# ohsnyt/bzip2-rust

Measured on NVIDIA B200. Metric: compress_MBps_level9_byte_identical, higher is better.
Workload: dtype u8

## Files before the change

bzip2_rust_b200/csrc/common.cuh:

```cuda
#pragma once
#include <cuda_runtime.h>
#include <stdint.h>
#include <stddef.h>
#include <mutex>
#include <string>
#include <vector>
#include <new>
#include "../../include/bz2b200.h"

typedef uint8_t u8;
typedef uint16_t u16;
typedef uint32_t u32;
typedef uint64_t u64;

#define BZ_CHECK(call)                                                                     \
    do {                                                                                   \
        cudaError_t e_ = (call);                                                           \
        if (e_ != cudaSuccess) {                                                           \
            ctx->fail(#call, e_, __FILE__, __LINE__);                                      \
            return BZ2B200_E_CUDA;                                                         \
        }                                                                                  \
    } while (0)

#define BZ_API_TRY try {
// ... 35 lines not shown
constexpr int BZ_TILE = BZ_THREADS * BZ_IPT;
constexpr int BZ_GROUP = 50;
constexpr int BZ_MAXSYM = 258;

struct Batch {
    int nblk;
    u32 stride;
    u32 tiles;
    u32 max_n;
    int nbits;
    const u8 *T;
    const u32 *len;
    u64 total_n;
};

enum KernelId { K_RADIX_HIST0, K_RADIX_SCAN, K_RADIX_SCATTER0, K_REF_PATH, K_BYTE_HIST, K_DIGIT_SCAN, K_SWEEP_GATHER, K_SWEEP_CARRY, K_SWEEP_LIST, K_INIT_RANKS, K_LIST_KEY, K_LIST_REFINE, K_REFINE_LOCAL, K_BWT_OUT, K_USED, K_MTF_SUMMARY, K_MTF_SCAN, K_MTF_EMIT, K_HUF_INIT, K_HUF_SELECT, K_HUF_LENGTHS, K_HUF_GBITS, K_HUF_LAYOUT, K_HUF_EMIT, K_RLE_SCAN, K_RLE_CHAIN, K_RLE_EMIT, K_CRC_PIECES, K_CRC_FINAL, K_CONCAT, K_FOOTER, K_DEC_MISC, K_DEC_MAGIC, K_DEC_HEADER, K_DEC_JUMPS, K_DEC_BOUNDS, K_DEC_SYMS, K_DEC_CHUNKS, K_DEC_EXPAND, K_DEC_CHUNK_SCAN, K_IBWT_CHASE, K_IBWT_RANK, K_IBWT_WRITE, K_DEC_RLE1_COUNT, K_DEC_RLE1_WRITE, K_COUNT };
static const char *const kKernelNames[] = { "k_radix_hist0", "k_radix_scan", "k_radix_scatter0", "k_ref_path", "k_byte_hist", "k_digit_scan", "k_sweep_gather", "k_sweep_carry", "k_sweep_list", "k_init_ranks", "k_list_key", "k_list_refine", "k_refine_local", "k_bwt_out", "k_used", "k_mtf_summary", "k_mtf_scan", "k_mtf_emit", "k_huf_init", "k_huf_select", "k_huf_lengths", "k_huf_gbits", "k_huf_layout", "k_huf_emit", "k_rle_scan", "k_rle_chain", "k_rle_emit", "k_crc_pieces", "k_crc_final", "k_concat", "k_footer", "k_dec_misc", "k_dec_find_magic", "k_dec_header", "k_dec_jumps", "k_dec_bounds", "k_dec_syms", "k_dec_chunks", "k_dec_expand", "k_dec_chunk_scan", "k_ibwt_chase", "k_ibwt_rank", "k_ibwt_write", "k_dec_rle1_count", "k_dec_rle1_write" };

struct KStat { double ms = 0; u64 launches = 0; u64 bytes = 0; };
struct PendingEv { int id; u64 bytes; cudaEvent_t a, b; };

struct Arrival {
    std::vector<cudaEvent_t> *ev;
    size_t chunk;
    size_t win_off;
    size_t waited;
};

struct ShardPlan {
    bool scanned = false;
    const u8 *d_win = nullptr; size_t win_lo = 0, win_len = 0, n_total = 0; int level = 0;
    bool planned = false;
// ... 215 lines not shown
```

bzip2_rust_b200/csrc/rle1.cu:

```cuda
#include "common.cuh"
#include <algorithm>
#include <stdlib.h>

namespace {

constexpr u32 CRC_POLY = 0x04C11DB7u;
constexpr int PIECE = 1024;
constexpr u32 NOQ = 0xFFFFFFFFu;

struct BlockRec {
    u32 s, e;
    u32 re;
    u32 g_last;
    u32 out_re;
    u32 out_g;
    u32 out_len;
    u32 last;
};

__host__ __device__ inline u32 gf_mul(u32 a, u32 b) {
    u32 r = 0;
    for (int i = 31; i >= 0; i--) {
        r = (r << 1) ^ ((r & 0x80000000u) ? CRC_POLY : 0u);
        if ((b >> i) & 1u) r ^= a;
// ... 48 lines not shown
        if (!((need >> lane) & 1u)) { v.a = -1; v.c = 0; }
#pragma unroll
        for (int o = 16; o; o >>= 1) {
            v.a = max(v.a, __shfl_xor_sync(0xffffffffu, v.a, o));
            v.c += __shfl_xor_sync(0xffffffffu, v.c, o);
        }
        ex.a = max(ex.a, v.a); ex.c += v.c;
        if (incm) break;
        hi -= 32;
    }
    Pair inc; inc.a = max(ex.a, agg.a); inc.c = ex.c + agg.c;
    if (lane == 0) st_vol64(st + t, pair_pack(2, inc));
    return ex;
}

struct ScanArgs {
    const u8 *x; u32 W;
    u32 *RS, *OUT, *LASTQ;
    u64 *st1, *st2;
    u32 *ticket;
};

constexpr int SC_IPT = 16;
constexpr int SC_TILE = BZ_THREADS * SC_IPT;

#ifndef BZ_SCAN_MINB
#define BZ_SCAN_MINB 5
#endif
__global__ void __launch_bounds__(BZ_THREADS, BZ_SCAN_MINB) k_rle_scan(ScanArgs a) {
    __shared__ u32 s_tile;
    __shared__ int wsi[8];
    __shared__ u32 wsu[8];
    __shared__ Pair s_ex1, s_ex2;
    const int tid = threadIdx.x;
    if (tid == 0) s_tile = atomicAdd(a.ticket, 1u);
    __syncthreads();
    const u32 t = s_tile, W = a.W;
    const u32 i0 = t * SC_TILE + tid * SC_IPT;
    u32 v[6];
    {
        uintptr_t addr = (uintptr_t)(a.x + i0) - 4;
        const u32 *gw = (const u32 *)(addr & ~(uintptr_t)3);
        const u32 mis = (u32)(addr & 3);
        long long j = (long long)i0 - 4 - (long long)mis;
        u32 w[7];
#pragma unroll
        for (int k = 0; k < 7; k++) {
            long long jk = j + 4 * k;
// ... 6 lines not shown
    int last = -1; u32 bdmask = 0;
#pragma unroll
    for (int r = 0; r < SC_IPT; r++) {
        u32 i = i0 + r;
        if (i < W && (i == 0 || XB(r) != XB(r - 1))) { last = (int)i; bdmask |= 1u << r; }
    }
    int tot1;
    int rs = block_excl_max(last, wsi, tot1);
    if (tid < 32) {
        Pair agg; agg.a = tot1; agg.c = 0;
        Pair ex = pair_lookback(a.st1, t, agg);
        if (tid == 0) s_ex1 = ex;
    }
    __syncthreads();
    rs = max(rs, s_ex1.a);
    u32 qmask = 0, litmask = 0, sum = 0;
    int lq = -1;
    const bool full = i0 + SC_IPT <= W;
    u32 rsv[SC_IPT];
#pragma unroll
    for (int r = 0; r < SC_IPT; r++) {
        u32 i = i0 + r;
        rsv[r] = 0;
        if (i < W) {
            if ((bdmask >> r) & 1u) rs = (int)i;
            rsv[r] = (u32)rs;
            u32 d = i - (u32)rs;
            u32 co = d - (d / 255u) * 255u;
            bool grp;
            if (co >= 3) grp = true;
            else {
                u32 c = XB(r);
                grp = (i - co) + 3 < W;
                if (co < 3) grp = grp && XB(r + 1) == c;
                if (co < 2) grp = grp && XB(r + 2) == c;
                if (co < 1) grp = grp && XB(r + 3) == c;
            }
            if (!grp) { litmask |= 1u << r; sum += 1; }
            else if (co == 0) { qmask |= 1u << r; sum += 5; lq = (int)i; }
        }
    }
    if (full) {
        uint4 *o = (uint4 *)(a.RS + i0);
#pragma unroll
        for (int k = 0; k < 4; k++) o[k] = make_uint4(rsv[4 * k], rsv[4 * k + 1], rsv[4 * k + 2], rsv[4 * k + 3]);
    } else {
#pragma unroll
        for (int r = 0; r < SC_IPT; r++) if (i0 + r < W) a.RS[i0 + r] = rsv[r];
    }
    int tq; u32 ts;
    int q = block_excl_max(lq, wsi, tq);
    u32 o = block_excl_sum(sum, wsu, ts);
    if (tid < 32) {
        Pair agg; agg.a = tq; agg.c = ts;
        Pair ex = pair_lookback(a.st2, t, agg);
        if (tid == 0) s_ex2 = ex;
    }
    __syncthreads();
    q = max(q, s_ex2.a);
    o += s_ex2.c;
    u32 ov[SC_IPT], qv[SC_IPT];
#pragma unroll
    for (int r = 0; r < SC_IPT; r++) {
        if ((qmask >> r) & 1u) q = (int)(i0 + r);
        ov[r] = o; qv[r] = q < 0 ? NOQ : (u32)q;
        o += ((litmask >> r) & 1u) + 5u * ((qmask >> r) & 1u);
        if (i0 + r == W - 1) a.OUT[W] = o;
    }
    if (full) {
        uint4 *po = (uint4 *)(a.OUT + i0), *pq = (uint4 *)(a.LASTQ + i0);
#pragma unroll
        for (int k = 0; k < 4; k++) {
            po[k] = make_uint4(ov[4 * k], ov[4 * k + 1], ov[4 * k + 2], ov[4 * k + 3]);
            pq[k] = make_uint4(qv[4 * k], qv[4 * k + 1], qv[4 * k + 2], qv[4 * k + 3]);
        }
    } else {
#pragma unroll
        for (int r = 0; r < SC_IPT; r++) if (i0 + r < W) { a.OUT[i0 + r] = ov[r]; a.LASTQ[i0 + r] = qv[r]; }
    }
#undef XB
}

struct ChainArgs {
    const u8 *x; const u32 *RS; const u32 *OUT; const u32 *LASTQ;
    u32 W;
    u32 B;
    u32 is_eof;
    u32 max_blocks;
    u32 max_out;
    u32 s0;
    u32 stop_at;
    u32 out_w;
    u32 off_from;
    BlockRec *rec; u32 *nrec; u32 *consumed;
};

__device__ u32 warp_lower_bound(const u32 *OUT, u32 lo, u32 hi, long long target) {
    int lane = threadIdx.x & 31;
    while (hi - lo > 32) {
        u32 step = (hi - lo + 31) / 32;
        u64 pp = (u64)lo + (u64)step * (u32)(lane + 1);
        u32 p = pp > hi ? hi : (u32)pp;
        bool ge = (long long)OUT[p] >= target;
        unsigned bal = __ballot_sync(0xffffffffu, ge);
        int f = __ffs(bal) - 1;
        u64 nh = (u64)lo + (u64)step * (u32)(f + 1);
        u32 new_hi = nh > hi ? hi : (u32)nh;
        u32 new_lo = f == 0 ? lo : lo + step * (u32)f + 1;
        lo = new_lo; hi = new_hi;
    }
    u32 p = lo + (u32)lane;
    bool ge = p <= hi && (long long)OUT[p] >= target;
    unsigned bal = __ballot_sync(0xffffffffu, ge);
    return lo + (u32)(__ffs(bal) - 1);
}

__device__ u32 run_end_from(const u32 *RS, u32 W, u32 s) {
    u32 key = RS[s];
    u32 d = 1;
    while (s + d < W && RS[s + d] == key && d < (1u << 30)) d <<= 1;
    u32 lo = s + (d >> 1) + 1, hi = (s + d < W) ? s + d : W;
    if (d == 1) lo = s + 1;
    while (lo < hi) {
        u32 mid = lo + (hi - lo) / 2;
        if (RS[mid] > key) hi = mid; else lo = mid + 1;
    }
    return lo;
}
__device__ u32 group_end(const u8 *x, u32 W, u32 q) {
    u8 c = x[q];
    u32 p = q + 4, lim = min(W, q + 255);
    while (p < lim && x[p] == c) p++;
    return p;
}
__device__ __forceinline__ u32 exit_cursor(u32 g, long long R) {
    if (R <= 1) return g + 1;
    return (R & 1) ? g + (u32)R : g + (u32)R + 1;
}

enum { PLAN_OK = 0, PLAN_STOP = 1, PLAN_SEARCH = 2 };
template <bool COOP>
__device__ __forceinline__ int plan_block(const ChainArgs &a, u32 s, BlockRec &r) {
    const u32 W = a.W, B = a.B;
    const u32 margin = a.is_eof ? 0u : 1024u;
    r.s = s; r.last = 0;
    u32 re = run_end_from(a.RS, W, s);
    if (!a.is_eof && re + margin > W) return PLAN_STOP;
    u32 Lc = re - s;
    u32 nfull = Lc / 255u, rem = Lc % 255u;
    u32 ng_avail = nfull + (rem >= 4 ? 1u : 0u);
    u32 jmax = (B - 1 + 4) / 5;
    u32 g, out_g;
    bool done = false;
    u32 e = 0;
    if (ng_avail > jmax) {
        g = s + 255u * jmax; out_g = 5u * jmax;
        e = g + 1;
        r.re = re; r.out_re = 0;
        done = true;
    } else {
        g = s + 255u * nfull + (rem >= 4 ? rem : 0u);
        out_g = 5u * ng_avail;
        r.re = re; r.out_re = out_g + (re - g);
    }
    bool has_group_after_off = ng_avail > 0 && g > a.off_from;
    if (!done) {
        long long off = (long long)r.out_re - (long long)a.OUT[re];
        long long target = (long long)B - 1 - off;
        u32 x1;
        u32 lq_m1 = NOQ, lq_p3 = NOQ;
        bool have_m1 = false, have_p3 = false;
        if ((long long)a.out_w < target) x1 = W + 1;
        else {
            long long need = target - (long long)a.OUT[re];
            u64 guess = (u64)re + (u64)(need > 0 ? need : 0);
            bool solved = false;
            if (need <= 0) { x1 = re; solved = true; }
            else if (COOP) {
                const int lane = threadIdx.x & 31;
                const long long wlo = (long long)guess - 15;
                const long long p = wlo + lane;
                const bool inb = p >= (long long)re && p <= (long long)W;
                const u32 o = inb ? a.OUT[p] : 0u;
                const u32 lqv = (p >= 0 && p < (long long)W) ? a.LASTQ[p] : NOQ;
                const unsigned bal = __ballot_sync(0xffffffffu, inb && (long long)o >= target);
                const unsigned inm = __ballot_sync(0xffffffffu, inb);
                if (bal) {
                    const int f = __ffs(bal) - 1;
                    const long long xp = wlo + f;
                    if (xp == (long long)re || (f > 0 && ((inm >> (f - 1)) & 1u))) {
                        x1 = (u32)xp; solved = true;
                        if (f >= 1) { lq_m1 = __shfl_sync(0xffffffffu, lqv, f - 1); have_m1 = true; }
                        const long long hl = (long long)min(x1 + 3, W - 1) - wlo;
                        if (hl >= 0 && hl < 32) { lq_p3 = __shfl_sync(0xffffffffu, lqv, (int)hl); have_p3 = true; }
                    }
                }
            }
            if (!solved) {
                if (guess <= W && (long long)a.OUT[guess] >= target && (long long)a.OUT[guess - 1] < target) x1 = (u32)guess;
                else if (COOP) {
                    u64 g64 = guess > W ? W : guess;
                    u32 lo_w = g64 > (u64)re + 512 ? (u32)g64 - 512u : re;
                    u32 hi_w = g64 + 512 < (u64)W ? (u32)g64 + 512u : W;
                    if ((long long)a.OUT[lo_w] < target && (long long)a.OUT[hi_w] >= target) x1 = warp_lower_bound(a.OUT, lo_w, hi_w, target);
                    else x1 = warp_lower_bound(a.OUT, re, W, target);
                } else {
                    u32 lo = re, hi = W;
                    while (lo < hi) {
                        u32 mid = lo + (hi - lo) / 2;
                        if ((long long)a.OUT[mid] >= target) hi = mid; else lo = mid + 1;
                    }
                    x1 = lo;
                }
            }
        }
        u32 gl = NOQ;
        if (x1 <= W) {
            u32 hiq = min(x1 + 3, W - 1);
            u32 q1_pre = x1 < W ? (have_p3 ? lq_p3 : a.LASTQ[hiq]) : NOQ;
            u32 qp_pre = x1 > re ? (have_m1 ? lq_m1 : a.LASTQ[x1 - 1]) : NOQ;
            if (x1 < W) {
                u32 q1 = q1_pre;
                if (q1 != NOQ && q1 >= x1 && q1 >= re && (long long)a.OUT[q1] + off == (long long)B - 1) {
                    u32 gp = g;
                    if (q1 > 0) {
                        u32 qp = a.LASTQ[q1 - 1];
                        if (qp != NOQ && qp >= re) gp = group_end(a.x, W, qp);
                    }
                    if (((q1 - gp) & 1u) == 1u) gl = q1;
                }
            }
            if (gl == NOQ && x1 > re) {
                u32 qp = qp_pre;
                if (qp != NOQ && qp >= re) gl = qp;
            }
        } else if (W > re) {
            u32 qp = a.LASTQ[W - 1];
            if (qp != NOQ && qp >= re) gl = qp;
        }
        if (gl != NOQ) {
            u32 out_gl = a.OUT[gl];
            g = group_end(a.x, W, gl);
            out_g = (u32)((long long)out_gl + off + 5);
            if (gl >= a.off_from) has_group_after_off = true;
        }
        long long R = (long long)B - (long long)out_g;
        e = exit_cursor(g, R);
    }
    if (a.is_eof) {
        u32 lim = has_group_after_off ? W - 1 : W - 2;
        if (W < 2 || e > lim || e > W) {
            e = W; r.last = 1;
            if (!done) {
                if (W > re) {
                    u32 qp = a.LASTQ[W - 1];
                    if (qp != NOQ && qp >= re) {
                        long long off = (long long)r.out_re - (long long)a.OUT[re];
                        g = group_end(a.x, W, qp);
                        out_g = (u32)((long long)a.OUT[qp] + off + 5);
                    }
                }
            } else {
                g = s + 255u * nfull + (rem >= 4 ? rem : 0u);
                out_g = 5u * ng_avail;
                r.out_re = out_g + (re - g);
            }
        }
    } else if (e + margin > W) {
        return PLAN_STOP;
    }
    r.e = e; r.g_last = g; r.out_g = out_g;
    r.out_len = out_g + (e - g);
    if (r.out_len > a.max_out) return PLAN_STOP;
    return PLAN_OK;
// ... 4 lines not shown
constexpr u32 CH_SEG = 128;
__host__ __device__ inline u32 tab_cap(u32 k) { return 32u * k + 256u; }
__host__ __device__ inline u32 tab_off(u32 k) { return 16u * k * (k - 1u) + 256u * (k - 1u); }
constexpr u32 TAB_ENTRIES = 16u * (CH_SEG + 1) * CH_SEG + 256u * CH_SEG;
constexpr u32 REC_BAD = 0xFFFFFFFFu;

struct ChainState { u32 nb, s, done, hits; };

struct TabArgs {
    ChainArgs a;
    ChainState *state;
    u32 *tlo, *tcnt;
    BlockRec *tab;
};

__device__ u32 lower_bound_out(const u32 *OUT, u32 lo, u32 hi, u64 target) {
    if ((u64)OUT[hi] < target) return hi + 1;
    while (lo < hi) {
        u32 mid = lo + (hi - lo) / 2;
        if ((u64)OUT[mid] >= target) hi = mid; else lo = mid + 1;
    }
    return lo;
}

__global__ void __launch_bounds__(128) k_rle_tab_bounds(TabArgs t) {
    const u32 k = blockIdx.x * 128 + threadIdx.x + 1;
    if (k > CH_SEG) return;
    const ChainState st = *t.state;
    t.tcnt[k] = 0;
    if (st.done || st.s >= t.a.W) return;
    const u32 W = t.a.W, B = t.a.B;
    const u64 base = t.a.OUT[st.s];
    u32 lo = lower_bound_out(t.a.OUT, st.s, W, base + (u64)k * (B - 10));
    if (lo > W) return;
    u32 hi = lower_bound_out(t.a.OUT, lo, W, base + (u64)k * (B + 15) + 1);
    if (hi > W) hi = W;
    u32 cap = tab_cap(k);
    if (hi - lo + 1 > cap) {
        u32 c = lower_bound_out(t.a.OUT, lo, hi, base + (u64)k * B + (5ull * k) / 2);
        u32 from = c > lo + cap / 2 ? c - cap / 2 : lo;
        if (from + cap - 1 > hi) from = hi + 1 - cap;
        lo = from; hi = from + cap - 1;
    }
    t.tlo[k] = lo; t.tcnt[k] = hi - lo + 1;
}

__global__ void __launch_bounds__(128) k_rle_tab_fill(TabArgs t) {
    const u32 k = blockIdx.y + 1;
    const u32 j = blockIdx.x * 128 + threadIdx.x;
    if (j >= t.tcnt[k]) return;
    const u32 s = t.tlo[k] + j;
    BlockRec r;
    r.out_len = REC_BAD;
    if (s < t.a.W) {
        ChainArgs a = t.a;
        a.out_w = a.OUT[a.W];
        if (plan_block<false>(a, s, r) != PLAN_OK) r.out_len = REC_BAD;
    }
    t.tab[tab_off(k) + j] = r;
}

__global__ void __launch_bounds__(32) k_rle_chain(TabArgs t) {
    ChainArgs a = t.a;
    const int lane = threadIdx.x;
    const u32 W = a.W;
    ChainState st = *t.state;
    if (st.done) return;
    a.out_w = a.OUT[W];
    u32 s = st.s, nb = st.nb, hits = st.hits;
    u32 span = a.B;
    bool finished = true;
    for (u32 k = 0;; k++) {
        if (!(s < W && s < a.stop_at && nb < a.max_blocks)) break;
        if (k > CH_SEG) { finished = false; break; }
        BlockRec r;
        bool have = false;
        if (t.tab && k >= 1) {
            u32 lo = t.tlo[k], cnt = t.tcnt[k];
            if (s >= lo && s - lo < cnt) {
                const uint4 *src = (const uint4 *)(t.tab + tab_off(k) + (s - lo));
                uint4 q0 = src[0], q1 = src[1];
                r.s = q0.x; r.e = q0.y; r.re = q0.z; r.g_last = q0.w; r.out_re = q1.x; r.out_g = q1.y; r.out_len = q1.z; r.last = q1.w;
                have = r.out_len != REC_BAD && r.s == s;
                hits += have ? 1u : 0u;
            }
        }
        if (!have) {
            {
                u64 c = (u64)s + (u64)span * (lane < 16 ? 1u : 2u);
                long long p = (long long)c - 1024 + (long long)(lane & 15) * 128;
                if (p >= 0 && (u64)p + 32 < (u64)W) {
                    prefetch_l2(a.OUT + p); prefetch_l2(a.OUT + p + 32); prefetch_l2(a.OUT + p + 64); prefetch_l2(a.OUT + p + 96);
                    prefetch_l2(a.LASTQ + p); prefetch_l2(a.LASTQ + p + 32); prefetch_l2(a.LASTQ + p + 64); prefetch_l2(a.LASTQ + p + 96);
                    prefetch_l2(a.RS + p); prefetch_l2(a.RS + p + 32); prefetch_l2(a.RS + p + 64); prefetch_l2(a.RS + p + 96);
                    prefetch_l2(a.x + p);
                }
            }
            if (plan_block<true>(a, s, r) != PLAN_OK) break;
        }
        if (lane == 0) a.rec[nb] = r;
        nb++;
        span = r.e - s;
        s = r.e;
    }
    if (lane == 0) {
        ChainState o; o.nb = nb; o.s = s; o.done = finished ? 1u : 0u; o.hits = hits;
        *t.state = o;
        *a.nrec = nb; *a.consumed = s;
    }
}

__global__ void __launch_bounds__(BZ_THREADS) k_rle_emit(const u8 *x, u32 W, const u32 *RS, const u32 *OUT,
                                                         const BlockRec *rec, u8 *T, u32 *len, u32 stride) {
    u32 k = blockIdx.y;
    BlockRec r = rec[k];
    u32 span = r.e - r.s;
    u32 base = blockIdx.x * BZ_TILE;
    if (base >= span) return;
    if (blockIdx.x == 0 && threadIdx.x == 0) len[k] = r.out_len;
    u8 *out = T + (size_t)k * stride;
    long long off = (long long)r.out_re - (long long)OUT[min(r.re, W)];
#pragma unroll 4
    for (int q = 0; q < BZ_IPT; q++) {
        u32 rel = base + q * BZ_THREADS + threadIdx.x;
        if (rel >= span) continue;
        u32 i = r.s + rel;
        u8 c = x[i];
        if (i >= r.g_last) {
            out[r.out_g + (i - r.g_last)] = c;
        } else if (i < r.re) {
            u32 j = (i - r.s) / 255u, cs = r.s + j * 255u;
            u32 cl = min(255u, r.re - cs);
            if (cl >= 4) {
                if (i == cs) {
                    u8 *o = out + 5u * j;
                    o[0] = c; o[1] = c; o[2] = c; o[3] = c; o[4] = (u8)(cl - 4);
                }
            } else out[5u * j + (i - cs)] = c;
        } else {
            u32 o0 = OUT[i], o1 = OUT[i + 1];
            u32 o = (u32)((long long)o0 + off);
            if (o1 - o0 == 1u) out[o] = c;
            else if (o1 != o0) {
                u32 ge = group_end(x, W, i);
                out[o] = c; out[o + 1] = c; out[o + 2] = c; out[o + 3] = c; out[o + 4] = (u8)(ge - i - 4);
            }
        }
    }
}

__global__ void __launch_bounds__(256) k_crc_pieces(const u8 *x, const u32 *spans, u32 span_stride, u32 s0, u32 e0,
                                                    u32 *part, u32 parts_stride, u32 xp ) {
    __shared__ u32 tab[256];
    __shared__ u32 red[256];
    make_crc_table(tab);
    u32 k = blockIdx.y;
    u32 s = spans ? spans[(size_t)k * span_stride] : s0, e = spans ? spans[(size_t)k * span_stride + 1] : e0;
    u32 span = e - s;
    u32 npieces = (span + PIECE - 1) / PIECE;
    u32 p = blockIdx.x * 256 + threadIdx.x;
    __syncthreads();
// ... 51 lines not shown
    do {                                                             \
        ctx->prof_end();                                             \
        cudaError_t e_ = cudaGetLastError();                         \
        if (e_ != cudaSuccess) { ctx->fail("kernel launch", e_, __FILE__, __LINE__); return BZ2B200_E_CUDA; } \
    } while (0)

int bz_rle1_window(bz2b200_ctx *ctx, const u8 *d_x, u32 W, int level, bool is_eof, u32 off_from, u32 max_blocks,
                   Batch &B, u32 *nblocks, u32 *consumed, std::vector<u32> *h_spans, bool plan_only, u32 stop_at,
                   int skip, u32 s0) {
    const bool skip_scan = skip & 1, skip_chain = skip & 2;
    cudaStream_t st = ctx->stream;
    u32 Bsz = (u32)level * 100000u - 19u;
    u32 max_n = Bsz + 8;
    u32 stride = ((max_n + 64 + BZ_TILE - 1) / BZ_TILE) * BZ_TILE;
    u32 tiles = (W + BZ_TILE - 1) / BZ_TILE;
    const size_t W4 = ((size_t)W + 1 + 3) & ~(size_t)3;
    BZ_CHECK(ctx->d_runflag.ensure(W4 * 4 * 3 + 64));
    u32 *RS = ctx->d_runflag.as<u32>();
    u32 *OUT = RS + W4;
    u32 *LASTQ = OUT + W4;
    const size_t state_bytes = ((size_t)tiles * 8 * 2 + 64 + 15) & ~(size_t)15;
    BZ_CHECK(ctx->d_misc.ensure(state_bytes + (size_t)max_blocks * sizeof(BlockRec) + 256));
    u64 *st1 = ctx->d_misc.as<u64>();
    u64 *st2 = st1 + tiles;
    u32 *ticket = (u32 *)(st2 + tiles);
    BlockRec *rec = (BlockRec *)(ctx->d_misc.as<u8>() + state_bytes);
    u32 *d_small = (u32 *)(rec + max_blocks);
    BZ_CHECK(ctx->h_small.ensure(64 + (size_t)max_blocks * sizeof(BlockRec)));

    if (!skip_scan && W > 0) {
        BZ_CHECK(cudaMemsetAsync(st1, 0, state_bytes, st));
        ScanArgs sa;
        sa.x = d_x; sa.W = W; sa.RS = RS; sa.OUT = OUT; sa.LASTQ = LASTQ; sa.st1 = st1; sa.st2 = st2; sa.ticket = ticket;
        if (!ctx->arrival) {
            ctx->prof_begin(K_RLE_SCAN, (u64)W * 13); k_rle_scan<<<tiles, BZ_THREADS, 0, st>>>(sa); LAUNCH_OK();
        } else {
            Arrival &A = *ctx->arrival;
            const size_t nev = A.ev->size();
            u32 launched = 0;
            while (launched < tiles) {
                if (A.waited < nev) { BZ_CHECK(cudaStreamWaitEvent(st, (*A.ev)[A.waited], 0)); A.waited++; }
                size_t have = A.waited >= nev ? (size_t)-1 : A.waited * A.chunk;
                size_t have_win = have > A.win_off ? have - A.win_off : 0;
                u32 upto = have_win >= W ? tiles : (have_win > 64 ? (u32)((have_win - 64) / SC_TILE) : 0u);
                if (upto > launched) {
                    ctx->prof_begin(K_RLE_SCAN, (u64)(upto - launched) * SC_TILE * 13);
                    k_rle_scan<<<upto - launched, BZ_THREADS, 0, st>>>(sa); LAUNCH_OK();
                    launched = upto;
                }
            }
        }
    }
    ChainArgs a;
    a.x = d_x; a.RS = RS; a.OUT = OUT; a.LASTQ = LASTQ; a.W = W; a.B = Bsz; a.is_eof = is_eof ? 1u : 0u;
    a.max_blocks = max_blocks; a.max_out = max_n; a.off_from = off_from; a.stop_at = stop_at; a.s0 = s0;
    a.rec = rec; a.nrec = d_small; a.consumed = d_small + 1;
    if (plan_only && skip_chain) { *nblocks = 0; *consumed = 0; return BZ2B200_OK; }
    if (!skip_chain) {
        static const bool use_tab = [] { const char *e = getenv("BZ2B200_CHAIN_TABLES"); return !e || atoi(e) != 0; }();
        BZ_CHECK(ctx->d_F.ensure(sizeof(ChainState) + 2 * (size_t)(CH_SEG + 1) * 4 + (size_t)TAB_ENTRIES * sizeof(BlockRec) + 256));
        TabArgs t;
        t.a = a;
        t.state = ctx->d_F.as<ChainState>();
        t.tlo = (u32 *)(t.state + 1);
        t.tcnt = t.tlo + (CH_SEG + 1);
        t.tab = use_tab ? (BlockRec *)(((uintptr_t)(t.tcnt + (CH_SEG + 1)) + 15) & ~(uintptr_t)15) : nullptr;
        ChainState st0; st0.nb = 0; st0.s = s0; st0.done = 0; st0.hits = 0;
        BZ_CHECK(cudaMemcpyAsync(t.state, &st0, sizeof st0, cudaMemcpyHostToDevice, st));
        u64 span_in = (u64)W - (u64)(s0 < W ? s0 : W);
// ... 17 lines not shown
    { int bits = 0; u32 v = max_n - 1; while (v) { bits++; v >>= 1; } B.nbits = bits; }
    if (nb == 0) return BZ2B200_OK;
    BZ_CHECK(ctx->d_T.ensure((size_t)nb * stride + 64));
    BZ_CHECK(ctx->d_len.ensure((size_t)nb * 4));
    BZ_CHECK(ctx->d_crc.ensure((size_t)nb * 4));
    BlockRec *hrec = (BlockRec *)(hs + 16);
    BZ_CHECK(cudaMemcpyAsync(hrec, rec, (size_t)nb * sizeof(BlockRec), cudaMemcpyDeviceToHost, st));
    BZ_CHECK(cudaStreamSynchronize(st));
    u32 max_span = 0;
    B.total_n = 0;
    for (u32 k = 0; k < nb; k++) B.total_n += hrec[k].out_len;
    for (u32 k = 0; k < nb; k++) max_span = hrec[k].e - hrec[k].s > max_span ? hrec[k].e - hrec[k].s : max_span;
    if (h_spans) { h_spans->clear(); for (u32 k = 0; k < nb; k++) { h_spans->push_back(hrec[k].s); h_spans->push_back(hrec[k].e); h_spans->push_back(hrec[k].out_len); h_spans->push_back(hrec[k].last); } }
    if (plan_only) return BZ2B200_OK;
    dim3 ge((max_span + BZ_TILE - 1) / BZ_TILE, nb);
    ctx->prof_begin(K_RLE_EMIT, (u64)max_span * nb * 2); k_rle_emit<<<ge, BZ_THREADS, 0, st>>>(d_x, W, RS, OUT, rec, ctx->d_T.as<u8>(), ctx->d_len.as<u32>(), stride);
    LAUNCH_OK();
    u32 max_pieces = (max_span + PIECE - 1) / PIECE;
    u32 parts_stride = (max_pieces + 255) / 256;
    BZ_CHECK(ctx->d_agg2.ensure((size_t)nb * parts_stride * 4 + 64));
    u32 xp = gf_pow_x8(PIECE), xp256 = gf_pow_x8((u64)PIECE * 256);
    dim3 gc(parts_stride, nb);
    ctx->prof_begin(K_CRC_PIECES, (u64)*consumed); k_crc_pieces<<<gc, 256, 0, st>>>(d_x, (const u32 *)rec, sizeof(BlockRec) / 4, 0, 0, ctx->d_agg2.as<u32>(), parts_stride, xp); LAUNCH_OK();
    ctx->prof_begin(K_CRC_FINAL, 0); k_crc_final<<<nb, 32, 0, st>>>((const u32 *)rec, sizeof(BlockRec) / 4, 0, 0, ctx->d_agg2.as<u32>(), parts_stride, xp256, ctx->d_crc.as<u32>()); LAUNCH_OK();
    B.T = ctx->d_T.as<u8>();
    B.len = ctx->d_len.as<u32>();
    return BZ2B200_OK;
}

int bz_crc_dev(bz2b200_ctx *ctx, const u8 *d_x, u32 n, u32 *d_crc_out) {
    cudaStream_t st = ctx->stream;
// ... 25 lines not shown
```

Measured before the change: 7393.

## Replace per-byte RLE1 scan arrays with a compact run list and binary search

The RLE1 scan no longer writes three per-byte u32 arrays (run start, output offset, last group start). It now emits a compact list of runs of length four or more, each with its start, end and output offset, found through a decoupled-lookback prefix sum. The chain planner and the emit kernel recover output offsets and group starts by binary search over this list. This removes roughly twelve bytes per input byte of global writes and later reads, at the cost of search latency in the serial chain planner and extra lookups per byte in emit.

Result: faster. 7566 (median of 6 runs) (+2.3%).

```diff
diff --git a/bzip2_rust_b200/csrc/common.cuh b/bzip2_rust_b200/csrc/common.cuh
--- a/bzip2_rust_b200/csrc/common.cuh
+++ b/bzip2_rust_b200/csrc/common.cuh
@@ -73,8 +73,8 @@
     u64 total_n;
 };
 
-enum KernelId { K_RADIX_HIST0, K_RADIX_SCAN, K_RADIX_SCATTER0, K_REF_PATH, K_BYTE_HIST, K_DIGIT_SCAN, K_SWEEP_GATHER, K_SWEEP_CARRY, K_SWEEP_LIST, K_INIT_RANKS, K_LIST_KEY, K_LIST_REFINE, K_REFINE_LOCAL, K_BWT_OUT, K_USED, K_MTF_SUMMARY, K_MTF_SCAN, K_MTF_EMIT, K_HUF_INIT, K_HUF_SELECT, K_HUF_LENGTHS, K_HUF_GBITS, K_HUF_LAYOUT, K_HUF_EMIT, K_RLE_SCAN, K_RLE_CHAIN, K_RLE_EMIT, K_CRC_PIECES, K_CRC_FINAL, K_CONCAT, K_FOOTER, K_DEC_MISC, K_DEC_MAGIC, K_DEC_HEADER, K_DEC_JUMPS, K_DEC_BOUNDS, K_DEC_SYMS, K_DEC_CHUNKS, K_DEC_EXPAND, K_DEC_CHUNK_SCAN, K_IBWT_CHASE, K_IBWT_RANK, K_IBWT_WRITE, K_DEC_RLE1_COUNT, K_DEC_RLE1_WRITE, K_COUNT };
-static const char *const kKernelNames[] = { "k_radix_hist0", "k_radix_scan", "k_radix_scatter0", "k_ref_path", "k_byte_hist", "k_digit_scan", "k_sweep_gather", "k_sweep_carry", "k_sweep_list", "k_init_ranks", "k_list_key", "k_list_refine", "k_refine_local", "k_bwt_out", "k_used", "k_mtf_summary", "k_mtf_scan", "k_mtf_emit", "k_huf_init", "k_huf_select", "k_huf_lengths", "k_huf_gbits", "k_huf_layout", "k_huf_emit", "k_rle_scan", "k_rle_chain", "k_rle_emit", "k_crc_pieces", "k_crc_final", "k_concat", "k_footer", "k_dec_misc", "k_dec_find_magic", "k_dec_header", "k_dec_jumps", "k_dec_bounds", "k_dec_syms", "k_dec_chunks", "k_dec_expand", "k_dec_chunk_scan", "k_ibwt_chase", "k_ibwt_rank", "k_ibwt_write", "k_dec_rle1_count", "k_dec_rle1_write" };
+enum KernelId { K_RADIX_HIST0, K_RADIX_SCAN, K_RADIX_SCATTER0, K_REF_PATH, K_BYTE_HIST, K_DIGIT_SCAN, K_SWEEP_GATHER, K_SWEEP_CARRY, K_SWEEP_LIST, K_INIT_RANKS, K_LIST_KEY, K_LIST_REFINE, K_REFINE_LOCAL, K_BWT_OUT, K_USED, K_MTF_SUMMARY, K_MTF_SCAN, K_MTF_EMIT, K_HUF_INIT, K_HUF_SELECT, K_HUF_LENGTHS, K_HUF_GBITS, K_HUF_LAYOUT, K_HUF_EMIT, K_RLE_RUNS, K_RLE_CHAIN, K_RLE_EMIT_RUNS, K_CRC_PIECES, K_CRC_FINAL, K_CONCAT, K_FOOTER, K_DEC_MISC, K_DEC_MAGIC, K_DEC_HEADER, K_DEC_JUMPS, K_DEC_BOUNDS, K_DEC_SYMS, K_DEC_CHUNKS, K_DEC_EXPAND, K_DEC_CHUNK_SCAN, K_IBWT_CHASE, K_IBWT_RANK, K_IBWT_WRITE, K_DEC_RLE1_COUNT, K_DEC_RLE1_WRITE, K_COUNT };
+static const char *const kKernelNames[] = { "k_radix_hist0", "k_radix_scan", "k_radix_scatter0", "k_ref_path", "k_byte_hist", "k_digit_scan", "k_sweep_gather", "k_sweep_carry", "k_sweep_list", "k_init_ranks", "k_list_key", "k_list_refine", "k_refine_local", "k_bwt_out", "k_used", "k_mtf_summary", "k_mtf_scan", "k_mtf_emit", "k_huf_init", "k_huf_select", "k_huf_lengths", "k_huf_gbits", "k_huf_layout", "k_huf_emit", "k_rle_runs", "k_rle_chain", "k_rle_emit_runs", "k_crc_pieces", "k_crc_final", "k_concat", "k_footer", "k_dec_misc", "k_dec_find_magic", "k_dec_header", "k_dec_jumps", "k_dec_bounds", "k_dec_syms", "k_dec_chunks", "k_dec_expand", "k_dec_chunk_scan", "k_ibwt_chase", "k_ibwt_rank", "k_ibwt_write", "k_dec_rle1_count", "k_dec_rle1_write" };
 
 struct KStat { double ms = 0; u64 launches = 0; u64 bytes = 0; };
 struct PendingEv { int id; u64 bytes; cudaEvent_t a, b; };
diff --git a/bzip2_rust_b200/csrc/rle1.cu b/bzip2_rust_b200/csrc/rle1.cu
--- a/bzip2_rust_b200/csrc/rle1.cu
+++ b/bzip2_rust_b200/csrc/rle1.cu
@@ -86,9 +86,37 @@
     return ex;
 }
 
+__device__ __forceinline__ u64 sum_lookback(u64 *st, u32 t, u64 agg) {
+    const int lane = threadIdx.x & 31;
+    const u64 PAY = (1ull << 62) - 1;
+    if (t == 0) { if (lane == 0) st_vol64(st, (2ull << 62) | agg); return 0; }
+    if (lane == 0) st_vol64(st + t, (1ull << 62) | agg);
+    u64 ex = 0;
+    for (int hi = (int)t - 1;;) {
+        int tt = hi - lane;
+        u64 w = tt >= 0 ? ld_vol64(st + tt) : (2ull << 62);
+        u32 f = (u32)(w >> 62);
+        u32 incm = __ballot_sync(0xffffffffu, f == 2);
+        u32 nrm = __ballot_sync(0xffffffffu, f == 0);
+        u32 need = incm ? ((2u << (__ffs(incm) - 1)) - 1u) : 0xffffffffu;
+        if (nrm & need) continue;
+        u64 v = ((need >> lane) & 1u) ? (w & PAY) : 0ull;
+#pragma unroll
+        for (int o = 16; o; o >>= 1) v += __shfl_xor_sync(0xffffffffu, v, o);
+        ex += v;
+        if (incm) break;
+        hi -= 32;
+    }
+    if (lane == 0) st_vol64(st + t, (2ull << 62) | (ex + agg));
+    return ex;
+}
+
+__host__ __device__ __forceinline__ u32 run_out_len(u32 L) { u32 r = L % 255u; return 5u * (L / 255u) + (r >= 4 ? 5u : r); }
+
 struct ScanArgs {
     const u8 *x; u32 W;
-    u32 *RS, *OUT, *LASTQ;
+    uint4 *runs;
+    u32 *hdr;
     u64 *st1, *st2;
     u32 *ticket;
 };
@@ -96,14 +124,12 @@
 constexpr int SC_IPT = 16;
 constexpr int SC_TILE = BZ_THREADS * SC_IPT;
 
-#ifndef BZ_SCAN_MINB
-#define BZ_SCAN_MINB 5
-#endif
-__global__ void __launch_bounds__(BZ_THREADS, BZ_SCAN_MINB) k_rle_scan(ScanArgs a) {
+__global__ void __launch_bounds__(BZ_THREADS) k_rle_runs(ScanArgs a) {
     __shared__ u32 s_tile;
     __shared__ int wsi[8];
     __shared__ u32 wsu[8];
-    __shared__ Pair s_ex1, s_ex2;
+    __shared__ Pair s_ex1;
+    __shared__ u64 s_ex2;
     const int tid = threadIdx.x;
     if (tid == 0) s_tile = atomicAdd(a.ticket, 1u);
     __syncthreads();
@@ -140,75 +166,141 @@
     }
     __syncthreads();
     rs = max(rs, s_ex1.a);
-    u32 qmask = 0, litmask = 0, sum = 0;
-    int lq = -1;
-    const bool full = i0 + SC_IPT <= W;
-    u32 rsv[SC_IPT];
+    const int rs_in = rs;
+    u32 endmask = 0, cnt = 0, sp = 0;
 #pragma unroll
     for (int r = 0; r < SC_IPT; r++) {
         u32 i = i0 + r;
-        rsv[r] = 0;
         if (i < W) {
             if ((bdmask >> r) & 1u) rs = (int)i;
-            rsv[r] = (u32)rs;
-            u32 d = i - (u32)rs;
-            u32 co = d - (d / 255u) * 255u;
-            bool grp;
-            if (co >= 3) grp = true;
-            else {
-                u32 c = XB(r);
-                grp = (i - co) + 3 < W;
-                if (co < 3) grp = grp && XB(r + 1) == c;
-                if (co < 2) grp = grp && XB(r + 2) == c;
-                if (co < 1) grp = grp && XB(r + 3) == c;
-            }
-            if (!grp) { litmask |= 1u << r; sum += 1; }
-            else if (co == 0) { qmask |= 1u << r; sum += 5; lq = (int)i; }
-        }
-    }
-    if (full) {
-        uint4 *o = (uint4 *)(a.RS + i0);
-#pragma unroll
-        for (int k = 0; k < 4; k++) o[k] = make_uint4(rsv[4 * k], rsv[4 * k + 1], rsv[4 * k + 2], rsv[4 * k + 3]);
+            u32 L = i + 1 - (u32)rs;
+            if (L >= 4 && (i + 1 == W || XB(r + 1) != XB(r))) {
+                endmask |= 1u << r;
+                cnt++; sp += L - run_out_len(L) + 1;
+            }
+        }
+    }
+    u32 tc, tsp;
+    u32 xc = block_excl_sum(cnt, wsu, tc);
+    u32 xsp = block_excl_sum(sp, wsu, tsp);
+    if (tid < 32) {
+        u64 ex = sum_lookback(a.st2, t, ((u64)tc << 31) | tsp);
+        if (tid == 0) s_ex2 = ex;
+    }
+    __syncthreads();
+    const u64 ex2 = s_ex2;
+    u32 idx = (u32)(ex2 >> 31) + xc;
+    u32 spb = (u32)(ex2 & 0x7fffffffu) + xsp;
+    rs = rs_in;
+#pragma unroll
+    for (int r = 0; r < SC_IPT; r++) {
+        if ((bdmask >> r) & 1u) rs = (int)(i0 + r);
+        if ((endmask >> r) & 1u) {
+            u32 s = (u32)rs, e = i0 + r + 1;
+            a.runs[1 + idx] = make_uint4(s, e, s - (spb - idx), 0u);
+            spb += e - s - run_out_len(e - s) + 1; idx++;
+        }
+    }
+    if (tid == 0) {
+        if (t == 0) a.runs[0] = make_uint4(0u, 0u, 0u, 0u);
+        if ((u64)(t + 1) * SC_TILE >= W) {
+            u32 n = (u32)(ex2 >> 31) + tc;
+            u32 out_w = W - ((u32)(ex2 & 0x7fffffffu) + tsp - n);
+            a.hdr[0] = n; a.hdr[1] = out_w;
+            a.runs[n + 1] = make_uint4(W, W, out_w, 0u);
+        }
+    }
+#undef XB
+}
+
+struct RunList {
+    const uint4 *r;
+    const u8 *x;
+    u32 W;
+    u32 n;
+};
+
+template <bool COOP, int F>
+__device__ __forceinline__ u32 rl_last_le(const RunList &L, u32 key) {
+    u32 lo = 0, hi = L.n + 1;
+    auto fld = [&](u32 k) -> u32 { return F == 0 ? L.r[k].x : L.r[k].z; };
+    if constexpr (COOP) {
+        const u32 lane = threadIdx.x & 31;
+        while (hi - lo >= 32) {
+            u32 step = (hi - lo + 31) / 32;
+            u32 p = min(hi, lo + step * (lane + 1));
+            u32 c = __popc(__ballot_sync(0xffffffffu, fld(p) <= key));
+            u32 nlo = c == 0 ? lo : min(hi, lo + step * c);
+            u32 nhi = c == 32 ? hi : min(hi, lo + step * (c + 1)) - 1;
+            lo = nlo; hi = nhi;
+        }
+        u32 p = lo + lane;
+        u32 c = __popc(__ballot_sync(0xffffffffu, p <= hi && fld(min(p, hi)) <= key));
+        return lo + c - 1;
     } else {
-#pragma unroll
-        for (int r = 0; r < SC_IPT; r++) if (i0 + r < W) a.RS[i0 + r] = rsv[r];
-    }
-    int tq; u32 ts;
-    int q = block_excl_max(lq, wsi, tq);
-    u32 o = block_excl_sum(sum, wsu, ts);
-    if (tid < 32) {
-        Pair agg; agg.a = tq; agg.c = ts;
-        Pair ex = pair_lookback(a.st2, t, agg);
-        if (tid == 0) s_ex2 = ex;
-    }
-    __syncthreads();
-    q = max(q, s_ex2.a);
-    o += s_ex2.c;
-    u32 ov[SC_IPT], qv[SC_IPT];
-#pragma unroll
-    for (int r = 0; r < SC_IPT; r++) {
-        if ((qmask >> r) & 1u) q = (int)(i0 + r);
-        ov[r] = o; qv[r] = q < 0 ? NOQ : (u32)q;
-        o += ((litmask >> r) & 1u) + 5u * ((qmask >> r) & 1u);
-        if (i0 + r == W - 1) a.OUT[W] = o;
-    }
-    if (full) {
-        uint4 *po = (uint4 *)(a.OUT + i0), *pq = (uint4 *)(a.LASTQ + i0);
-#pragma unroll
-        for (int k = 0; k < 4; k++) {
-            po[k] = make_uint4(ov[4 * k], ov[4 * k + 1], ov[4 * k + 2], ov[4 * k + 3]);
-            pq[k] = make_uint4(qv[4 * k], qv[4 * k + 1], qv[4 * k + 2], qv[4 * k + 3]);
-        }
-    } else {
-#pragma unroll
-        for (int r = 0; r < SC_IPT; r++) if (i0 + r < W) { a.OUT[i0 + r] = ov[r]; a.LASTQ[i0 + r] = qv[r]; }
-    }
-#undef XB
-}
+        while (lo < hi) {
+            u32 mid = lo + (hi - lo + 1) / 2;
+            if (fld(mid) <= key) lo = mid; else hi = mid - 1;
+        }
+        return lo;
+    }
+}
+
+__device__ __forceinline__ u32 rl_out(const uint4 q, u32 x) {
+    if (x < q.y) {
+        u32 d = x - q.x, j = d / 255u, co = d - 255u * j, cl = min(255u, q.y - q.x - 255u * j);
+        return q.z + 5u * j + (cl >= 4 ? (co ? 5u : 0u) : co);
+    }
+    return q.z + run_out_len(q.y - q.x) + (x - q.y);
+}
+
+template <bool COOP>
+__device__ __forceinline__ u32 out_at(const RunList &L, u32 x) { return rl_out(L.r[rl_last_le<COOP, 0>(L, x)], x); }
+
+template <bool COOP>
+__device__ u32 last_group_start(const RunList &L, u32 x) {
+    u32 k = rl_last_le<COOP, 0>(L, x);
+    if (k == 0) return NOQ;
+    const uint4 q = L.r[k];
+    const u32 len = q.y - q.x;
+    u32 j;
+    if (x < q.y) {
+        j = (x - q.x) / 255u;
+        if (min(255u, len - 255u * j) < 4) j--;
+    } else j = len / 255u + (len % 255u >= 4 ? 1u : 0u) - 1u;
+    return q.x + 255u * j;
+}
+
+template <bool COOP>
+__device__ u32 run_end_from(const RunList &L, u32 s) {
+    const uint4 q = L.r[rl_last_le<COOP, 0>(L, s)];
+    if (s < q.y) return q.y;
+    const u8 c = L.x[s];
+    u32 p = s + 1;
+    while (p < L.W && L.x[p] == c) p++;
+    return p;
+}
+
+template <bool COOP>
+__device__ u32 lower_bound_out(const RunList &L, long long target) {
+    if (target <= 0) return 0;
+    if (target > 0xFFFFFFFFll) return L.W + 1;
+    const u32 k = rl_last_le<COOP, 2>(L, (u32)(target - 1));
+    if (k == L.n + 1) return L.W + 1;
+    const uint4 q = L.r[k];
+    const u32 need = (u32)target - q.z, len = q.y - q.x, ol = run_out_len(len);
+    if (need <= ol) {
+        u32 j = (need - 1) / 5u;
+        return min(255u, len - 255u * j) >= 4 ? q.x + 255u * j + 1u : q.x + 255u * j + (need - 5u * j);
+    }
+    return q.y + (need - ol);
+}
+__device__ __forceinline__ u32 clamp_lb(u32 x, u32 lo, u32 hi) { return x < lo ? lo : (x > hi ? hi + 1 : x); }
 
 struct ChainArgs {
-    const u8 *x; const u32 *RS; const u32 *OUT; const u32 *LASTQ;
+    const u8 *x;
+    RunList runs;
+    const u32 *hdr;
     u32 W;
     u32 B;
     u32 is_eof;
@@ -220,39 +312,8 @@
     u32 off_from;
     BlockRec *rec; u32 *nrec; u32 *consumed;
 };
-
-__device__ u32 warp_lower_bound(const u32 *OUT, u32 lo, u32 hi, long long target) {
-    int lane = threadIdx.x & 31;
-    while (hi - lo > 32) {
-        u32 step = (hi - lo + 31) / 32;
-        u64 pp = (u64)lo + (u64)step * (u32)(lane + 1);
-        u32 p = pp > hi ? hi : (u32)pp;
-        bool ge = (long long)OUT[p] >= target;
-        unsigned bal = __ballot_sync(0xffffffffu, ge);
-        int f = __ffs(bal) - 1;
-        u64 nh = (u64)lo + (u64)step * (u32)(f + 1);
-        u32 new_hi = nh > hi ? hi : (u32)nh;
-        u32 new_lo = f == 0 ? lo : lo + step * (u32)f + 1;
-        lo = new_lo; hi = new_hi;
-    }
-    u32 p = lo + (u32)lane;
-    bool ge = p <= hi && (long long)OUT[p] >= target;
-    unsigned bal = __ballot_sync(0xffffffffu, ge);
-    return lo + (u32)(__ffs(bal) - 1);
-}
-
-__device__ u32 run_end_from(const u32 *RS, u32 W, u32 s) {
-    u32 key = RS[s];
-    u32 d = 1;
-    while (s + d < W && RS[s + d] == key && d < (1u << 30)) d <<= 1;
-    u32 lo = s + (d >> 1) + 1, hi = (s + d < W) ? s + d : W;
-    if (d == 1) lo = s + 1;
-    while (lo < hi) {
-        u32 mid = lo + (hi - lo) / 2;
-        if (RS[mid] > key) hi = mid; else lo = mid + 1;
-    }
-    return lo;
-}
+__device__ __forceinline__ void load_run_header(ChainArgs &a) { a.runs.n = a.hdr[0]; a.out_w = a.hdr[1]; }
+
 __device__ u32 group_end(const u8 *x, u32 W, u32 q) {
     u8 c = x[q];
     u32 p = q + 4, lim = min(W, q + 255);
@@ -267,10 +328,11 @@
 enum { PLAN_OK = 0, PLAN_STOP = 1, PLAN_SEARCH = 2 };
 template <bool COOP>
 __device__ __forceinline__ int plan_block(const ChainArgs &a, u32 s, BlockRec &r) {
+    const RunList &L = a.runs;
     const u32 W = a.W, B = a.B;
     const u32 margin = a.is_eof ? 0u : 1024u;
     r.s = s; r.last = 0;
-    u32 re = run_end_from(a.RS, W, s);
+    u32 re = run_end_from<COOP>(L, s);
     if (!a.is_eof && re + margin > W) return PLAN_STOP;
     u32 Lc = re - s;
     u32 nfull = Lc / 255u, rem = Lc % 255u;
@@ -291,81 +353,33 @@
     }
     bool has_group_after_off = ng_avail > 0 && g > a.off_from;
     if (!done) {
-        long long off = (long long)r.out_re - (long long)a.OUT[re];
+        long long off = (long long)r.out_re - (long long)out_at<COOP>(L, re);
         long long target = (long long)B - 1 - off;
-        u32 x1;
-        u32 lq_m1 = NOQ, lq_p3 = NOQ;
-        bool have_m1 = false, have_p3 = false;
-        if ((long long)a.out_w < target) x1 = W + 1;
-        else {
-            long long need = target - (long long)a.OUT[re];
-            u64 guess = (u64)re + (u64)(need > 0 ? need : 0);
-            bool solved = false;
-            if (need <= 0) { x1 = re; solved = true; }
-            else if (COOP) {
-                const int lane = threadIdx.x & 31;
-                const long long wlo = (long long)guess - 15;
-                const long long p = wlo + lane;
-                const bool inb = p >= (long long)re && p <= (long long)W;
-                const u32 o = inb ? a.OUT[p] : 0u;
-                const u32 lqv = (p >= 0 && p < (long long)W) ? a.LASTQ[p] : NOQ;
-                const unsigned bal = __ballot_sync(0xffffffffu, inb && (long long)o >= target);
-                const unsigned inm = __ballot_sync(0xffffffffu, inb);
-                if (bal) {
-                    const int f = __ffs(bal) - 1;
-                    const long long xp = wlo + f;
-                    if (xp == (long long)re || (f > 0 && ((inm >> (f - 1)) & 1u))) {
-                        x1 = (u32)xp; solved = true;
-                        if (f >= 1) { lq_m1 = __shfl_sync(0xffffffffu, lqv, f - 1); have_m1 = true; }
-                        const long long hl = (long long)min(x1 + 3, W - 1) - wlo;
-                        if (hl >= 0 && hl < 32) { lq_p3 = __shfl_sync(0xffffffffu, lqv, (int)hl); have_p3 = true; }
-                    }
-                }
-            }
-            if (!solved) {
-                if (guess <= W && (long long)a.OUT[guess] >= target && (long long)a.OUT[guess - 1] < target) x1 = (u32)guess;
-                else if (COOP) {
-                    u64 g64 = guess > W ? W : guess;
-                    u32 lo_w = g64 > (u64)re + 512 ? (u32)g64 - 512u : re;
-                    u32 hi_w = g64 + 512 < (u64)W ? (u32)g64 + 512u : W;
-                    if ((long long)a.OUT[lo_w] < target && (long long)a.OUT[hi_w] >= target) x1 = warp_lower_bound(a.OUT, lo_w, hi_w, target);
-                    else x1 = warp_lower_bound(a.OUT, re, W, target);
-                } else {
-                    u32 lo = re, hi = W;
-                    while (lo < hi) {
-                        u32 mid = lo + (hi - lo) / 2;
-                        if ((long long)a.OUT[mid] >= target) hi = mid; else lo = mid + 1;
-                    }
-                    x1 = lo;
-                }
-            }
-        }
+        u32 x1 = (long long)a.out_w < target ? W + 1
+                                             : clamp_lb(lower_bound_out<COOP>(L, target), re, W);
         u32 gl = NOQ;
         if (x1 <= W) {
-            u32 hiq = min(x1 + 3, W - 1);
-            u32 q1_pre = x1 < W ? (have_p3 ? lq_p3 : a.LASTQ[hiq]) : NOQ;
-            u32 qp_pre = x1 > re ? (have_m1 ? lq_m1 : a.LASTQ[x1 - 1]) : NOQ;
             if (x1 < W) {
-                u32 q1 = q1_pre;
-                if (q1 != NOQ && q1 >= x1 && q1 >= re && (long long)a.OUT[q1] + off == (long long)B - 1) {
+                u32 q1 = last_group_start<COOP>(L, min(x1 + 3, W - 1));
+                if (q1 != NOQ && q1 >= x1 && q1 >= re && (long long)out_at<COOP>(L, q1) + off == (long long)B - 1) {
                     u32 gp = g;
                     if (q1 > 0) {
-                        u32 qp = a.LASTQ[q1 - 1];
+                        u32 qp = last_group_start<COOP>(L, q1 - 1);
                         if (qp != NOQ && qp >= re) gp = group_end(a.x, W, qp);
                     }
                     if (((q1 - gp) & 1u) == 1u) gl = q1;
                 }
             }
             if (gl == NOQ && x1 > re) {
-                u32 qp = qp_pre;
+                u32 qp = last_group_start<COOP>(L, x1 - 1);
                 if (qp != NOQ && qp >= re) gl = qp;
             }
         } else if (W > re) {
-            u32 qp = a.LASTQ[W - 1];
+            u32 qp = last_group_start<COOP>(L, W - 1);
             if (qp != NOQ && qp >= re) gl = qp;
         }
         if (gl != NOQ) {
-            u32 out_gl = a.OUT[gl];
+            u32 out_gl = out_at<COOP>(L, gl);
             g = group_end(a.x, W, gl);
             out_g = (u32)((long long)out_gl + off + 5);
             if (gl >= a.off_from) has_group_after_off = true;
@@ -379,11 +393,11 @@
             e = W; r.last = 1;
             if (!done) {
                 if (W > re) {
-                    u32 qp = a.LASTQ[W - 1];
+                    u32 qp = last_group_start<COOP>(L, W - 1);
                     if (qp != NOQ && qp >= re) {
-                        long long off = (long long)r.out_re - (long long)a.OUT[re];
+                        long long off = (long long)r.out_re - (long long)out_at<COOP>(L, re);
                         g = group_end(a.x, W, qp);
-                        out_g = (u32)((long long)a.OUT[qp] + off + 5);
+                        out_g = (u32)((long long)out_at<COOP>(L, qp) + off + 5);
                     }
                 }
             } else {
@@ -418,30 +432,23 @@
     BlockRec *tab;
 };
 
-__device__ u32 lower_bound_out(const u32 *OUT, u32 lo, u32 hi, u64 target) {
-    if ((u64)OUT[hi] < target) return hi + 1;
-    while (lo < hi) {
-        u32 mid = lo + (hi - lo) / 2;
-        if ((u64)OUT[mid] >= target) hi = mid; else lo = mid + 1;
-    }
-    return lo;
-}
-
 __global__ void __launch_bounds__(128) k_rle_tab_bounds(TabArgs t) {
     const u32 k = blockIdx.x * 128 + threadIdx.x + 1;
     if (k > CH_SEG) return;
     const ChainState st = *t.state;
     t.tcnt[k] = 0;
     if (st.done || st.s >= t.a.W) return;
+    load_run_header(t.a);
+    const RunList &L = t.a.runs;
     const u32 W = t.a.W, B = t.a.B;
-    const u64 base = t.a.OUT[st.s];
-    u32 lo = lower_bound_out(t.a.OUT, st.s, W, base + (u64)k * (B - 10));
+    const u64 base = out_at<false>(L, st.s);
+    u32 lo = clamp_lb(lower_bound_out<false>(L, (long long)(base + (u64)k * (B - 10))), st.s, W);
     if (lo > W) return;
-    u32 hi = lower_bound_out(t.a.OUT, lo, W, base + (u64)k * (B + 15) + 1);
+    u32 hi = clamp_lb(lower_bound_out<false>(L, (long long)(base + (u64)k * (B + 15) + 1)), lo, W);
     if (hi > W) hi = W;
     u32 cap = tab_cap(k);
     if (hi - lo + 1 > cap) {
-        u32 c = lower_bound_out(t.a.OUT, lo, hi, base + (u64)k * B + (5ull * k) / 2);
+        u32 c = clamp_lb(lower_bound_out<false>(L, (long long)(base + (u64)k * B + (5ull * k) / 2)), lo, hi);
         u32 from = c > lo + cap / 2 ? c - cap / 2 : lo;
         if (from + cap - 1 > hi) from = hi + 1 - cap;
         lo = from; hi = from + cap - 1;
@@ -458,7 +465,7 @@
     r.out_len = REC_BAD;
     if (s < t.a.W) {
         ChainArgs a = t.a;
-        a.out_w = a.OUT[a.W];
+        load_run_header(a);
         if (plan_block<false>(a, s, r) != PLAN_OK) r.out_len = REC_BAD;
     }
     t.tab[tab_off(k) + j] = r;
@@ -470,7 +477,7 @@
     const u32 W = a.W;
     ChainState st = *t.state;
     if (st.done) return;
-    a.out_w = a.OUT[W];
+    if (st.s < W) load_run_header(a);
     u32 s = st.s, nb = st.nb, hits = st.hits;
     u32 span = a.B;
     bool finished = true;
@@ -490,16 +497,9 @@
             }
         }
         if (!have) {
-            {
-                u64 c = (u64)s + (u64)span * (lane < 16 ? 1u : 2u);
-                long long p = (long long)c - 1024 + (long long)(lane & 15) * 128;
-                if (p >= 0 && (u64)p + 32 < (u64)W) {
-                    prefetch_l2(a.OUT + p); prefetch_l2(a.OUT + p + 32); prefetch_l2(a.OUT + p + 64); prefetch_l2(a.OUT + p + 96);
-                    prefetch_l2(a.LASTQ + p); prefetch_l2(a.LASTQ + p + 32); prefetch_l2(a.LASTQ + p + 64); prefetch_l2(a.LASTQ + p + 96);
-                    prefetch_l2(a.RS + p); prefetch_l2(a.RS + p + 32); prefetch_l2(a.RS + p + 64); prefetch_l2(a.RS + p + 96);
-                    prefetch_l2(a.x + p);
-                }
-            }
+            u64 c = (u64)s + (u64)span * (lane < 16 ? 1u : 2u);
+            long long p = (long long)c - 1024 + (long long)(lane & 15) * 128;
+            if (p >= 0 && (u64)p + 128 <= (u64)W) prefetch_l2(a.x + p);
             if (plan_block<true>(a, s, r) != PLAN_OK) break;
         }
         if (lane == 0) a.rec[nb] = r;
@@ -514,22 +514,33 @@
     }
 }
 
-__global__ void __launch_bounds__(BZ_THREADS) k_rle_emit(const u8 *x, u32 W, const u32 *RS, const u32 *OUT,
-                                                         const BlockRec *rec, u8 *T, u32 *len, u32 stride) {
-    u32 k = blockIdx.y;
-    BlockRec r = rec[k];
-    u32 span = r.e - r.s;
-    u32 base = blockIdx.x * BZ_TILE;
+__global__ void __launch_bounds__(BZ_THREADS) k_rle_emit_runs(RunList L, const u32 *hdr, const BlockRec *rec, u8 *T,
+                                                              u32 *len, u32 stride) {
+    __shared__ u32 s_k0, s_k1, s_outre;
+    const u32 k = blockIdx.y;
+    const BlockRec r = rec[k];
+    const u32 span = r.e - r.s, base = blockIdx.x * BZ_TILE;
     if (base >= span) return;
     if (blockIdx.x == 0 && threadIdx.x == 0) len[k] = r.out_len;
+    L.n = hdr[0];
     u8 *out = T + (size_t)k * stride;
-    long long off = (long long)r.out_re - (long long)OUT[min(r.re, W)];
+    const u32 t0 = r.s + base, t1 = min(r.e, t0 + BZ_TILE);
+    const u32 g0 = max(t0, r.re), g1 = min(t1, r.g_last);
+    const u32 warp = threadIdx.x >> 5;
+    if (g0 < g1) {
+        if (warp == 0) { u32 v = rl_last_le<true, 0>(L, g0); if ((threadIdx.x & 31) == 0) s_k0 = v; }
+        if (warp == 1) { u32 v = rl_last_le<true, 0>(L, g1 - 1); if ((threadIdx.x & 31) == 0) s_k1 = v; }
+        if (warp == 2) { u32 v = out_at<true>(L, r.re); if ((threadIdx.x & 31) == 0) s_outre = v; }
+    }
+    __syncthreads();
+    const u32 k1 = s_k1;
+    const u32 off = r.out_re - s_outre;
+    u32 kc = s_k0;
 #pragma unroll 4
     for (int q = 0; q < BZ_IPT; q++) {
-        u32 rel = base + q * BZ_THREADS + threadIdx.x;
-        if (rel >= span) continue;
-        u32 i = r.s + rel;
-        u8 c = x[i];
+        u32 i = t0 + q * BZ_THREADS + threadIdx.x;
+        if (i >= t1) break;
+        u8 c = L.x[i];
         if (i >= r.g_last) {
             out[r.out_g + (i - r.g_last)] = c;
         } else if (i < r.re) {
@@ -542,13 +553,21 @@
                 }
             } else out[5u * j + (i - cs)] = c;
         } else {
-            u32 o0 = OUT[i], o1 = OUT[i + 1];
-            u32 o = (u32)((long long)o0 + off);
-            if (o1 - o0 == 1u) out[o] = c;
-            else if (o1 != o0) {
-                u32 ge = group_end(x, W, i);
-                out[o] = c; out[o + 1] = c; out[o + 2] = c; out[o + 3] = c; out[o + 4] = (u8)(ge - i - 4);
-            }
+            u32 lo = kc, hi = k1;
+            while (lo < hi) {
+                u32 mid = lo + (hi - lo + 1) / 2;
+                if (L.r[mid].x <= i) lo = mid; else hi = mid - 1;
+            }
+            kc = lo;
+            const uint4 R = L.r[kc];
+            if (i < R.y) {
+                u32 d = i - R.x, j = d / 255u, co = d - 255u * j, cl = min(255u, R.y - R.x - 255u * j);
+                u32 o = R.z + 5u * j + off;
+                if (cl < 4) out[o + co] = c;
+                else if (co == 0) {
+                    out[o] = c; out[o + 1] = c; out[o + 2] = c; out[o + 3] = c; out[o + 4] = (u8)(cl - 4);
+                }
+            } else out[R.z + run_out_len(R.y - R.x) + (i - R.y) + off] = c;
         }
     }
 }
@@ -630,11 +649,9 @@
     u32 max_n = Bsz + 8;
     u32 stride = ((max_n + 64 + BZ_TILE - 1) / BZ_TILE) * BZ_TILE;
     u32 tiles = (W + BZ_TILE - 1) / BZ_TILE;
-    const size_t W4 = ((size_t)W + 1 + 3) & ~(size_t)3;
-    BZ_CHECK(ctx->d_runflag.ensure(W4 * 4 * 3 + 64));
-    u32 *RS = ctx->d_runflag.as<u32>();
-    u32 *OUT = RS + W4;
-    u32 *LASTQ = OUT + W4;
+    BZ_CHECK(ctx->d_runflag.ensure(((size_t)W / 4 + 3) * sizeof(uint4)));
+    u32 *hdr = ctx->d_runflag.as<u32>();
+    uint4 *runs = ctx->d_runflag.as<uint4>() + 1;
     const size_t state_bytes = ((size_t)tiles * 8 * 2 + 64 + 15) & ~(size_t)15;
     BZ_CHECK(ctx->d_misc.ensure(state_bytes + (size_t)max_blocks * sizeof(BlockRec) + 256));
     u64 *st1 = ctx->d_misc.as<u64>();
@@ -647,9 +664,9 @@
     if (!skip_scan && W > 0) {
         BZ_CHECK(cudaMemsetAsync(st1, 0, state_bytes, st));
         ScanArgs sa;
-        sa.x = d_x; sa.W = W; sa.RS = RS; sa.OUT = OUT; sa.LASTQ = LASTQ; sa.st1 = st1; sa.st2 = st2; sa.ticket = ticket;
+        sa.x = d_x; sa.W = W; sa.runs = runs; sa.hdr = hdr; sa.st1 = st1; sa.st2 = st2; sa.ticket = ticket;
         if (!ctx->arrival) {
-            ctx->prof_begin(K_RLE_SCAN, (u64)W * 13); k_rle_scan<<<tiles, BZ_THREADS, 0, st>>>(sa); LAUNCH_OK();
+            ctx->prof_begin(K_RLE_RUNS, W); k_rle_runs<<<tiles, BZ_THREADS, 0, st>>>(sa); LAUNCH_OK();
         } else {
             Arrival &A = *ctx->arrival;
             const size_t nev = A.ev->size();
@@ -660,15 +677,15 @@
                 size_t have_win = have > A.win_off ? have - A.win_off : 0;
                 u32 upto = have_win >= W ? tiles : (have_win > 64 ? (u32)((have_win - 64) / SC_TILE) : 0u);
                 if (upto > launched) {
-                    ctx->prof_begin(K_RLE_SCAN, (u64)(upto - launched) * SC_TILE * 13);
-                    k_rle_scan<<<upto - launched, BZ_THREADS, 0, st>>>(sa); LAUNCH_OK();
+                    ctx->prof_begin(K_RLE_RUNS, (u64)(upto - launched) * SC_TILE);
+                    k_rle_runs<<<upto - launched, BZ_THREADS, 0, st>>>(sa); LAUNCH_OK();
                     launched = upto;
                 }
             }
         }
     }
     ChainArgs a;
-    a.x = d_x; a.RS = RS; a.OUT = OUT; a.LASTQ = LASTQ; a.W = W; a.B = Bsz; a.is_eof = is_eof ? 1u : 0u;
+    a.x = d_x; a.runs.r = runs; a.runs.x = d_x; a.runs.W = W; a.runs.n = 0; a.hdr = hdr; a.out_w = 0; a.W = W; a.B = Bsz; a.is_eof = is_eof ? 1u : 0u;
     a.max_blocks = max_blocks; a.max_out = max_n; a.off_from = off_from; a.stop_at = stop_at; a.s0 = s0;
     a.rec = rec; a.nrec = d_small; a.consumed = d_small + 1;
     if (plan_only && skip_chain) { *nblocks = 0; *consumed = 0; return BZ2B200_OK; }
@@ -716,7 +733,8 @@
     if (h_spans) { h_spans->clear(); for (u32 k = 0; k < nb; k++) { h_spans->push_back(hrec[k].s); h_spans->push_back(hrec[k].e); h_spans->push_back(hrec[k].out_len); h_spans->push_back(hrec[k].last); } }
     if (plan_only) return BZ2B200_OK;
     dim3 ge((max_span + BZ_TILE - 1) / BZ_TILE, nb);
-    ctx->prof_begin(K_RLE_EMIT, (u64)max_span * nb * 2); k_rle_emit<<<ge, BZ_THREADS, 0, st>>>(d_x, W, RS, OUT, rec, ctx->d_T.as<u8>(), ctx->d_len.as<u32>(), stride);
+    ctx->prof_begin(K_RLE_EMIT_RUNS, (u64)B.total_n + *consumed);
+    k_rle_emit_runs<<<ge, BZ_THREADS, 0, st>>>(a.runs, hdr, rec, ctx->d_T.as<u8>(), ctx->d_len.as<u32>(), stride);
     LAUNCH_OK();
     u32 max_pieces = (max_span + PIECE - 1) / PIECE;
     u32 parts_stride = (max_pieces + 255) / 256;
```
